# geoeo/ORB_SLAM3_V1.0

Measured on AMD Instinct MI355X. Metric: frames/sec ORB extract+match, 752x480 8-level 1000-feat; bit-exact kp/desc, higher is better.
Workload: dtype u8

## Files before the change

orb_slam3_v1.0_amd/csrc/fast_common.h:

```cpp
#pragma once
#include <hip/hip_runtime.h>
#include <stdint.h>

namespace orbfe {

constexpr int kFastTW = 64, kFastTH = 32;

constexpr int kFusedPyramidMinFrames = 0;

__device__ __forceinline__ bool arc9(uint32_t m)
{
    uint32_t m2 = m | (m << 16);
    uint32_t r = m2 & (m2 >> 1);
    r &= r >> 2;
    r &= r >> 4;
    r &= m2 >> 8;
    return (r & 0xffffu) != 0;
}

__device__ __forceinline__ bool corner_at_global(const uint8_t* __restrict__ img, int pitch, int x, int y, int th)
{
    const int8_t dy[16] = {3, 3, 2, 1, 0, -1, -2, -3, -3, -3, -2, -1, 0, 1, 2, 3};
    const int8_t dx[16] = {0, 1, 2, 3, 3, 3, 2, 1, 0, -1, -2, -3, -3, -3, -2, -1};
    const int v = img[(size_t)y * pitch + x];
    uint32_t mb = 0, md = 0;
#pragma unroll
    for (int k = 0; k < 16; k++) {
        const int d = (int)img[(size_t)(y + dy[k]) * pitch + x + dx[k]] - v;
        mb |= (uint32_t)(d > th) << k;
        md |= (uint32_t)(d < -th) << k;
    }
    return arc9(mb) || arc9(md);
}

}
```

orb_slam3_v1.0_amd/csrc/kernels_fast.hip:

```cpp
#include <cstdlib>

#include "launch.h"
#include "device_math.h"
#include "fast_common.h"

namespace orbfe {

constexpr int kImgW = kFastTW + 8, kImgH = kFastTH + 8;
constexpr int kScH = kFastTH + 2;
constexpr int kScW = kFastTW + 2;
constexpr int kScPitch = kImgW;
constexpr int kScoreOfs = 3 * kImgW + 3;
constexpr int kMaxTileCand = (kFastTW / 2) * (kFastTH / 2);
constexpr int kTmpH = kFastTH + 4;
constexpr int kQCap = 2304;
static_assert(kQCap >= kScH * kScW && kQCap % 2 == 0, "stage A geometry");

typedef unsigned short u16x2 __attribute__((ext_vector_type(2)));


__device__ __forceinline__ unsigned long long mask_le_u32(uint32_t x, uint32_t bound)
{
    unsigned long long m;
    asm("v_cmp_le_u32_e64 %0, %1, %2" : "=s"(m) : "v"(x), "s"(bound));
    return m;
}

__device__ __forceinline__ unsigned long long mask_ge_u32(uint32_t x, uint32_t bound)
{
    unsigned long long m;
    asm("v_cmp_ge_u32_e64 %0, %1, %2" : "=s"(m) : "v"(x), "s"(bound));
    return m;
}
__device__ __forceinline__ unsigned long long mask_gt_u32(uint32_t a, uint32_t b)
{
    unsigned long long m;
    asm("v_cmp_gt_u32_e64 %0, %1, %2" : "=s"(m) : "v"(a), "v"(b));
    return m;
}
__device__ __forceinline__ uint32_t select_by_mask(unsigned long long mask, uint32_t a, uint32_t b)
{
    uint32_t r;
    asm("v_cndmask_b32_e64 %0, %1, %2, %3" : "=v"(r) : "v"(b), "v"(a), "s"(mask));
    return r;
}
__device__ __forceinline__ void masked_lds_add(unsigned long long mask, uint32_t addr, uint32_t v)
{
    unsigned long long save;
    asm volatile("s_and_saveexec_b64 %0, %1\n\tds_add_u32 %2, %3\n\ts_mov_b64 exec, %0" : "=&s"(save) : "s"(mask), "v"(addr), "v"(v) : "scc", "memory");
}
__device__ __forceinline__ void masked_lds_write_b32(unsigned long long mask, uint32_t addr, uint32_t v)
{
    unsigned long long save;
    asm volatile("s_and_saveexec_b64 %0, %1\n\tds_write_b32 %2, %3\n\ts_mov_b64 exec, %0" : "=&s"(save) : "s"(mask), "v"(addr), "v"(v) : "scc", "memory");
}
__device__ __forceinline__ unsigned long long mask_lt_i32(uint32_t a, int b, bool vbound = false)
{
    unsigned long long m;
    if (vbound) asm("v_cmp_lt_i32_e64 %0, %1, %2" : "=s"(m) : "v"(a), "v"(b));
    else asm("v_cmp_lt_i32_e64 %0, %1, %2" : "=s"(m) : "v"(a), "s"(b));
    return m;
}
__device__ __forceinline__ void masked_lds_write_b8(unsigned long long mask, uint32_t addr, uint32_t v)
{
    unsigned long long save;
    asm volatile("s_and_saveexec_b64 %0, %1\n\tds_write_b8 %2, %3\n\ts_mov_b64 exec, %0" : "=&s"(save) : "s"(mask), "v"(addr), "v"(v) : "scc", "memory");
}
__device__ __forceinline__ void masked_lds_write_b16(unsigned long long mask, uint32_t addr, uint32_t v)
{
    unsigned long long save;
    asm volatile("s_and_saveexec_b64 %0, %1\n\tds_write_b16 %2, %3\n\ts_mov_b64 exec, %0" : "=&s"(save) : "s"(mask), "v"(addr), "v"(v) : "scc", "memory");
}
__device__ __forceinline__ void lds_add(uint32_t* addr, uint32_t v)
{
    asm volatile("ds_add_u32 %0, %1" : : "v"((uint32_t)(uintptr_t)addr), "v"(v) : "memory");
}

__device__ __forceinline__ uint32_t lds_add_rtn(uint32_t* addr, uint32_t v)
{
    uint32_t old;
    asm volatile("ds_add_rtn_u32 %0, %1, %2\n\ts_waitcnt lgkmcnt(0)" : "=&v"(old) : "v"((uint32_t)(uintptr_t)addr), "v"(v) : "memory");
    return old;
}

__device__ __forceinline__ uint32_t min16(uint32_t a, uint32_t b)
{
    uint32_t r;
    asm("v_min_u16 %0, %1, %2" : "=v"(r) : "v"(a), "v"(b));
    return r;
}
__device__ __forceinline__ uint32_t max16(uint32_t a, uint32_t b)
{
    uint32_t r;
    asm("v_max_u16 %0, %1, %2" : "=v"(r) : "v"(a), "v"(b));
    return r;
}
__device__ __forceinline__ uint32_t sub16(uint32_t a, uint32_t b)
{
    uint32_t r;
    asm("v_sub_u16 %0, %1, %2" : "=v"(r) : "v"(a), "v"(b));
    return r;
}
__device__ __forceinline__ uint32_t maxi16(uint32_t a, uint32_t b)
{
    uint32_t r;
    asm("v_max_i16 %0, %1, %2" : "=v"(r) : "v"(a), "v"(b));
    return r;
}

template <bool DARK>
__device__ __forceinline__ uint32_t arc_extreme(const uint32_t (&p)[16])
{
    auto lo = [](uint32_t a, uint32_t b) { return DARK ? max16(a, b) : min16(a, b); };
    auto hi = [](uint32_t a, uint32_t b) { return DARK ? min16(a, b) : max16(a, b); };
    uint32_t m2[8], m4[8], a[8];
#pragma unroll
    for (int j = 0; j < 8; j++) m2[j] = lo(p[2 * j + 1], p[(2 * j + 2) & 15]);
#pragma unroll
    for (int j = 0; j < 8; j++) m4[j] = lo(m2[j], m2[(j + 1) & 7]);
#pragma unroll
    for (int j = 0; j < 8; j++) {
        const uint32_t core = lo(m4[j], m4[(j + 2) & 7]);
        a[j] = lo(core, hi(p[2 * j], p[(2 * j + 9) & 15]));
    }
#pragma unroll
    for (int st = 4; st >= 1; st >>= 1)
#pragma unroll
        for (int k = 0; k < st; k++) a[k] = hi(a[k], a[k + st]);
    return a[0];
}
__device__ __forceinline__ uint32_t arc_max_of_min(const uint32_t (&p)[16]) { return arc_extreme<false>(p); }
__device__ __forceinline__ uint32_t arc_min_of_max(const uint32_t (&p)[16]) { return arc_extreme<true>(p); }

__device__ __forceinline__ unsigned long long mask_th_i16(int th, uint32_t m)
{
    unsigned long long r;
    asm("v_cmp_lt_i16_e64 %0, %1, %2" : "=s"(r) : "s"(th), "v"(m));
    return r;
}

__device__ __forceinline__ int queue_slot1(uint32_t m, int th, unsigned long long mask, uint32_t entry, int stepV, int qNext)
{
    unsigned long long save;
    uint32_t tmp;
    int cnt;
    asm volatile("v_cmp_lt_i16_e32 vcc, %8, %3\n\t"
                 "s_and_b64 vcc, vcc, %4\n\t"
                 "s_and_saveexec_b64 %0, vcc\n\t"
                 "v_mbcnt_lo_u32_b32 %1, vcc_lo, 0\n\t"
                 "v_mbcnt_hi_u32_b32 %1, vcc_hi, %1\n\t"
                 "v_mad_i32_i24 %1, %1, %6, %7\n\t"
                 "ds_write_b16 %1, %5\n\t"
                 "s_mov_b64 exec, %0\n\t"
                 "s_bcnt1_i32_b64 %2, vcc"
                 : "=&s"(save), "=&v"(tmp), "=s"(cnt)
                 : "v"(m), "s"(mask), "v"(entry), "v"(stepV), "s"(qNext), "s"(th)
                 : "vcc", "scc", "memory");
    return cnt;
}

template <int MODE, bool BUILD>
__global__ __launch_bounds__(256) void fast_blur_kernel(const PipelineDesc* __restrict__ P,
                                                        const uint32_t* __restrict__ tileInfo, int tileBase,
                                                        const uint32_t* __restrict__ tabs,
                                                        const uint8_t* __restrict__ gray0, size_t gray0FrameStride,
// ... 41 lines not shown
    const int tid = threadIdx.x;
    const int lane = tid & 63;
    if (tid < 4) sCnt[tid] = 0;
    if (tid < 3) sQ[tid] = 0;
    if (tid < kFastTH) sRow[tid] = 0;

    int bXa = 0, bNX = 0, bYa = 0, bNY = 0;
    uint32_t bXt = 0, bYt = 0;
    if constexpr (BUILD) {
        const uint32_t* own = tabs + L.ownOff;
        const int tX = (int)(ti & 0xfffu), tY = (int)((ti >> 12) & 0xfffu);
        bXa = (int)own[tX];
        bNX = (int)own[tX + 1] - bXa;
        bYa = (int)own[L.tilesX + 1 + tY];
        bNY = (int)own[L.tilesX + 2 + tY] - bYa;
        const LevelDesc& D = P->lv[l + 1];
        if (lane < bNX) bXt = tabs[D.xtabOff + (size_t)(bXa + lane)];
        if (lane < bNY) bYt = tabs[D.ytabOff + (size_t)(bYa + lane)];
    }

    if (aligned) {
        if (tid < 14 * (kImgW / 4)) {
            const int r0 = tid / (kImgW / 4);
            const int c4 = tid - r0 * (kImgW / 4);
            const int gx = x0 - 4 + 4 * c4;
            const bool colIn = gx >= 0 && gx < w;
            uint32_t wv[3];
            if (y0 >= 4 && y0 + kFastTH + 4 <= h) {
                uint32_t off = __umul24((unsigned)(y0 - 4 + r0), (unsigned)spitch) + (unsigned)gx;
                const uint32_t step = 14u * (unsigned)spitch;
#pragma unroll
                for (int k = 0; k < 3; k++) {
                    wv[k] = 0;
                    if (colIn && r0 + 14 * k < kImgH) wv[k] = *reinterpret_cast<const uint32_t*>(src + off);
                    off += step;
                }
            } else {
#pragma unroll
                for (int k = 0; k < 3; k++) {
                    const int r = r0 + 14 * k;
                    wv[k] = 0;
                    if (colIn && r < kImgH)
                        wv[k] = *reinterpret_cast<const uint32_t*>(src + (size_t)reflect_near(y0 - 4 + r, h) * spitch + gx);
                }
            }
#pragma unroll
            for (int k = 0; k < 3; k++) {
                const int r = r0 + 14 * k;
                if (colIn && r < kImgH) *reinterpret_cast<uint32_t*>(&sImg[r][4 * c4]) = wv[k];
            }
        }
        const int cR = w - x0 + 4;
        const bool patchL = x0 == 0, patchR = cR + 1 < kImgW;
        if (patchL || patchR) {
            __syncthreads();
            if (tid < kImgH) {
                if (patchL) {
                    sImg[tid][2] = sImg[tid][6];
                    sImg[tid][3] = sImg[tid][5];
                }
            } else if (tid >= 64 && tid < 64 + kImgH) {
                if (patchR) {
                    sImg[tid - 64][cR] = sImg[tid - 64][cR - 2];
                    sImg[tid - 64][cR + 1] = sImg[tid - 64][cR - 3];
                }
            }
        }
    } else {
        for (int e = tid; e < kImgH * (kImgW / 4); e += 256) {
            const int r = e / (kImgW / 4);
            const int c4 = e - r * (kImgW / 4);
            const uint8_t* row = src + (size_t)reflect_near(y0 - 4 + r, h) * spitch;
            uint32_t wv = 0;
#pragma unroll
            for (int i = 0; i < 4; i++) wv |= (uint32_t)row[reflect_near(x0 - 4 + 4 * c4 + i, w)] << (8 * i);
            *reinterpret_cast<uint32_t*>(&sImg[r][4 * c4]) = wv;
        }
    }
    __syncthreads();

    if constexpr (BUILD) {
        static_assert(kFastTH == 32, "eight owned rows per wave at most");
        const LevelDesc& D = P->lv[l + 1];
        if (lane < bNX && bNY > 0) {
            const uint32_t wx = bXt >> 16, wxc = 2048u - wx;
            const uint8_t* sp = &sImg[0][0] + ((int)(bXt & 0xffffu) - (x0 - 4));
            uint8_t* dcol = ws + D.imgOff + (size_t)f * D.imgFrameStride + (uint32_t)(bYa * D.pitch + bXa + lane);
            const int q = __builtin_amdgcn_readfirstlane(tid >> 6);
            uint32_t top[8], bot[8], wy[8];
#pragma unroll
            for (int k = 0; k < 8; k++) {
                const uint32_t yt = (uint32_t)__builtin_amdgcn_readlane((int)bYt, min(q + 4 * k, bNY - 1));
                const uint8_t* pr = sp + ((int)(yt & 0xffffu) - (y0 - 4)) * kImgW;
                wy[k] = yt >> 16;
                top[k] = __umul24(pr[0], wxc) + __umul24(pr[1], wx);
                bot[k] = __umul24(pr[kImgW], wxc) + __umul24(pr[kImgW + 1], wx);
            }
#pragma unroll
            for (int k = 0; k < 8; k++) {
                const uint32_t v = __umul24(top[k], 2048u - wy[k]) + __umul24(bot[k], wy[k]) + (1u << 21);
                if (q + 4 * k < bNY) dcol[(uint32_t)((q + 4 * k) * D.pitch)] = (uint8_t)(v >> 22);
            }
        }
    }

    if constexpr ((MODE & 1) != 0) {
    for (int e = tid; e < (kTmpH / 2) * (kFastTW / 4); e += 256) {
        const int j = e / (kFastTW / 4);
        const int xl = (e - j * (kFastTW / 4)) * 4;
        uint32_t o[2][4];
#pragma unroll
        for (int half = 0; half < 2; half++) {
            const uint32_t* rowp = reinterpret_cast<const uint32_t*>(&sImg[2 * j + half + 2][xl]);
            const uint32_t w0 = rowp[0], w1 = rowp[1], w2 = rowp[2];
            o[half][0] = __builtin_amdgcn_udot4(w1, 0x00163E58u, __builtin_amdgcn_udot4(w0, 0x3E160000u, 0u, false), false);
            o[half][1] = __builtin_amdgcn_udot4(w1, 0x163E583Eu, __builtin_amdgcn_udot4(w0, 0x16000000u, 0u, false), false);
            o[half][2] = __builtin_amdgcn_udot4(w2, 0x00000016u, __builtin_amdgcn_udot4(w1, 0x3E583E16u, 0u, false), false);
            o[half][3] = __builtin_amdgcn_udot4(w2, 0x0000163Eu, __builtin_amdgcn_udot4(w1, 0x583E1600u, 0u, false), false);
        }
        uint4 pk;
        pk.x = o[0][0] | (o[1][0] << 16);
        pk.y = o[0][1] | (o[1][1] << 16);
        pk.z = o[0][2] | (o[1][2] << 16);
        pk.w = o[0][3] | (o[1][3] << 16);
        *reinterpret_cast<uint4*>(&sTmp[j][xl]) = pk;
    }
    __syncthreads();
    }

    const int wv = __builtin_amdgcn_readfirstlane(tid >> 6);
    if (wv >= 2) {
        if constexpr ((MODE & 2) != 0)
            for (int e = tid - 128; e < (kScH + 1) * (kScPitch / 4); e += 128) reinterpret_cast<uint32_t*>(&sScore[0][0])[e] = 0;
        if constexpr ((MODE & 1) != 0) {
            uint8_t* dst = ws + L.blurOff + (size_t)f * L.blurFrameStride;
            const int dpitch = L.pitch;
            const int xl = (tid & 15) * 4;
#pragma unroll 1
            for (int yp = (tid - 128) >> 4; yp < kFastTH / 2; yp += 8) {
                const int gy = y0 + 2 * yp, gx = x0 + xl;
                if (gy < h && gx < w) {
                    const uint4 p0 = *reinterpret_cast<const uint4*>(&sTmp[yp][xl]);
                    const uint4 p1 = *reinterpret_cast<const uint4*>(&sTmp[yp + 1][xl]);
                    const uint4 p2 = *reinterpret_cast<const uint4*>(&sTmp[yp + 2][xl]);
                    const uint32_t c0[4] = {p0.x, p0.y, p0.z, p0.w}, c1[4] = {p1.x, p1.y, p1.z, p1.w}, c2[4] = {p2.x, p2.y, p2.z, p2.w};
                    uint32_t ev[4], od[4];
#pragma unroll
                    for (int i = 0; i < 4; i++) {
                        const u16x2 a = __builtin_bit_cast(u16x2, c0[i]), b = __builtin_bit_cast(u16x2, c1[i]), c = __builtin_bit_cast(u16x2, c2[i]);
                        uint32_t acc = __builtin_amdgcn_udot2(a, __builtin_bit_cast(u16x2, 0x003E0016u), 32768u, false);
                        acc = __builtin_amdgcn_udot2(b, __builtin_bit_cast(u16x2, 0x003E0058u), acc, false);
                        ev[i] = __builtin_amdgcn_udot2(c, __builtin_bit_cast(u16x2, 0x00000016u), acc, false);
                        acc = __builtin_amdgcn_udot2(a, __builtin_bit_cast(u16x2, 0x00160000u), 32768u, false);
                        acc = __builtin_amdgcn_udot2(b, __builtin_bit_cast(u16x2, 0x0058003Eu), acc, false);
                        od[i] = __builtin_amdgcn_udot2(c, __builtin_bit_cast(u16x2, 0x0016003Eu), acc, false);
                    }
                    const uint32_t outE = __builtin_amdgcn_perm(ev[1], ev[0], 0x0c0c0602u) |
                                          (__builtin_amdgcn_perm(ev[3], ev[2], 0x0c0c0602u) << 16);
                    const uint32_t outO = __builtin_amdgcn_perm(od[1], od[0], 0x0c0c0602u) |
                                          (__builtin_amdgcn_perm(od[3], od[2], 0x0c0c0602u) << 16);
                    uint8_t* drow = dst + (size_t)gy * dpitch;
                    const bool odd = gy + 1 < h;
                    if (gx + 3 < w) {
                        *reinterpret_cast<uint32_t*>(drow + gx) = outE;
                        if (odd) *reinterpret_cast<uint32_t*>(drow + dpitch + gx) = outO;
                    } else {
                        for (int i = 0; gx + i < w; i++) {
                            drow[gx + i] = (uint8_t)(outE >> (8 * i));
                            if (odd) drow[dpitch + gx + i] = (uint8_t)(outO >> (8 * i));
                        }
                    }
                }
            }
        }
    } else if constexpr ((MODE & 2) != 0) {
        constexpr int kRowsA = kScH / 2;
        static_assert(2 * kRowsA == kScH && kScW == 66, "stage A geometry");
        const int R0 = wv ? 3 + kRowsA : 3;
        const int cLo = max(3, kEdge + 1 - (x0 - 4)), cHi = min(kScW + 2, w - kEdge - 1 - (x0 - 4));
        const int rLo = max(3, kEdge + 1 - (y0 - 4)), rHi = min(kScH + 2, h - kEdge - 1 - (y0 - 4));
        const uint32_t cSpan = (uint32_t)max(cHi - cLo, -1), rSpan = (uint32_t)max(rHi - rLo, -1);
        const bool anyValid = cSpan != 0xffffffffu && rSpan != 0xffffffffu;
        const unsigned long long colOK = anyValid ? mask_le_u32((uint32_t)(lane + 3 - cLo), cSpan) : 0ull;
        const int qStep = wv ? -2 : 2;
// ... 130 lines not shown
            if (mPre == 0) continue;
            const uint8_t* sp = &sScore[0][0] + (e - kScoreOfs);
            const uint32_t sc = sp[0];
            const uint32_t n0 = max16(max16((uint32_t)sp[-kScPitch - 1], (uint32_t)sp[-kScPitch]), (uint32_t)sp[-kScPitch + 1]);
            const uint32_t n1 = max16(max16((uint32_t)sp[-1], (uint32_t)sp[1]), (uint32_t)sp[kScPitch - 1]);
            const uint32_t n2 = max16((uint32_t)sp[kScPitch], (uint32_t)sp[kScPitch + 1]);
            const uint32_t nmax = max16(max16(n0, n1), n2);
            const unsigned long long mHi = mask_ge_u32(sc, (uint32_t)iniTh);
            const unsigned long long mKeep = mPre & mask_gt_u32(sc, nmax);
            const unsigned long long mPreHi = mPre & mHi, mKeepHi = mKeep & mHi;
            nPreW += (uint32_t)__popcll(mPre);
            nPreHiW += (uint32_t)__popcll(mPreHi);
            nKeepHiW += (uint32_t)__popcll(mKeepHi);
            masked_lds_add(mPre, rowLds + 4u * oy, select_by_mask(mHi, 0x10001u, 1u));
            if (mKeep) {
                uint32_t wbase = 0;
                if (lane == 0) wbase = lds_add_rtn(&sCnt[0], (uint32_t)__popcll(mKeep));
                wbase = __builtin_amdgcn_readfirstlane(wbase);
                const uint32_t rank = __builtin_amdgcn_mbcnt_hi((uint32_t)(mKeep >> 32), __builtin_amdgcn_mbcnt_lo((uint32_t)mKeep, 0u));
                masked_lds_write_b32(mKeep, candLds + 4u * (wbase + rank), pack_cand(x0 + (int)ox, y0 + (int)oy, (int)sc));
            }
        }
        if (lane == 0) {
            if (nPreW) lds_add(&sCnt[2], nPreW);
            if (nPreHiW) lds_add(&sCnt[3], nPreHiW);
            if (nKeepHiW) lds_add(&sCnt[1], nKeepHiW);
        }
        asm volatile("s_waitcnt lgkmcnt(0)" ::: "memory");
    }
    __syncthreads();

    }

    if (tid < kFastTH) {
        const uint32_t v = sRow[tid];
        tileRows[((size_t)f * P->totalTiles + tile) * kFastTH + tid] = (uint16_t)((v & 0xffu) | ((v >> 16) << 8));
    }

    uint32_t* cnt = counters + ((size_t)f * nL + l) * kCntWords;
    const uint32_t nTile = sCnt[0];
    if (tid == 0) {
        uint32_t base = 0;
        if constexpr ((MODE & 256) != 0) base = (uint32_t)tile * 8u;
        else if (nTile) base = atomicAdd(&cnt[kCntCand], nTile);
        if (sCnt[1]) atomicAdd(&cnt[kCntHigh], sCnt[1]);
        if (sCnt[2]) atomicAdd(&cnt[kCntPreLow], sCnt[2]);
        if (sCnt[3]) atomicAdd(&cnt[kCntPreHigh], sCnt[3]);
        sBase = base;
    }
    __syncthreads();
    if (nTile) {
        const uint32_t base = sBase;
        uint32_t* out = cand + L.candOff + (size_t)f * L.candCap;
        for (uint32_t i = tid; i < nTile; i += 256) {
            if (base + i < (uint32_t)L.candCap) out[base + i] = sCand[i];
            else atomicOr(&cnt[kCntStatus], (uint32_t)kFlagCandOverflow);
        }
    }
}

void fast_tiles_for(int w, int h, int* tx, int* ty)
{
    *tx = (w + kFastTW - 1) / kFastTW;
    *ty = (h + kFastTH - 1) / kFastTH;
}

bool fast_next_level_fits(const uint32_t* xtab, const uint32_t* ytab, int sw, int sh, int dw, int dh, uint32_t* own)
{
    int tx, ty;
    fast_tiles_for(sw, sh, &tx, &ty);
    bool ok = true;
    auto fill = [&](const uint32_t* tab, int srcN, int dstN, int tile, int nTiles, uint32_t* o) {
        int p = 0;
        for (int t = 0; t <= nTiles; t++) {
            while (p < dstN && (int)(tab[p] & 0xffffu) < t * tile) p++;
            o[t] = (uint32_t)(t == nTiles ? dstN : p);
            if (t > 0 && o[t] - o[t - 1] > 64u) ok = false;
        }
        for (int i = 0; i < dstN; i++)
            if ((int)(tab[i] & 0xffffu) + 1 > srcN - 1 || (i > 0 && (tab[i] & 0xffffu) < (tab[i - 1] & 0xffffu))) ok = false;
    };
    fill(xtab, sw, dw, kFastTW, tx, own);
    fill(ytab, sh, dh, kFastTH, ty, own + tx + 1);
    return ok;
}

uint32_t fast_tile_info(int level, int tileX, int tileY) { return ((uint32_t)level << 24) | ((uint32_t)tileY << 12) | (uint32_t)tileX; }

void launch_fast_blur(hipStream_t s, int frames, int tileBase, int nTiles, bool buildNext, const PipelineDesc* dP,
                      const uint32_t* dTileInfo, const uint32_t* dTabs, const uint8_t* gray0, size_t gray0FrameStride, int gray0Pitch,
                      int gray0Aligned4, uint8_t* ws, uint32_t* cand, uint32_t* counters, uint16_t* tileRows)
{
    dim3 block(256);
    dim3 grid(frames, nTiles);
    if (buildNext) {
        hipLaunchKernelGGL((fast_blur_kernel<3, true>), grid, block, 0, s, dP, dTileInfo, tileBase, dTabs, gray0, gray0FrameStride,
                           gray0Pitch, gray0Aligned4, ws, cand, counters, tileRows);
        return;
    }
#define ORBFE_LAUNCH_FB(M)                                                                                                      \
    hipLaunchKernelGGL((fast_blur_kernel<M, false>), grid, block, 0, s, dP, dTileInfo, tileBase, dTabs, gray0, gray0FrameStride, \
                       gray0Pitch, gray0Aligned4, ws, cand, counters, tileRows)
#ifdef ORBFE_ABLATION
    static const int mode = [] {
        const char* e = getenv("ORBFE_FAST_MODE");
        return e ? atoi(e) & 1023 : 3;
    }();
    switch (mode) {
    case 0: ORBFE_LAUNCH_FB(0); break;
    case 1: ORBFE_LAUNCH_FB(1); break;
    case 2: ORBFE_LAUNCH_FB(2); break;
    case 6: ORBFE_LAUNCH_FB(6); break;
    case 10: ORBFE_LAUNCH_FB(10); break;
    case 26: ORBFE_LAUNCH_FB(26); break;
    case 67: ORBFE_LAUNCH_FB(67); break;
    case 195: ORBFE_LAUNCH_FB(195); break;
    case 259: ORBFE_LAUNCH_FB(259); break;
    case 515: ORBFE_LAUNCH_FB(515); break;
    case 42: ORBFE_LAUNCH_FB(42); break;
    default: ORBFE_LAUNCH_FB(3); break;
    }
#else
    ORBFE_LAUNCH_FB(3);
#endif
#undef ORBFE_LAUNCH_FB
}

}
```

orb_slam3_v1.0_amd/csrc/orbfe_host.cpp:

```cpp
#include <atomic>
#include <cmath>
#include <cstdio>
#include <cstdlib>
#include <cstring>
#include <map>
#include <mutex>
#include <new>
#include <condition_variable>
#include <functional>
#include <string>
#include <thread>
#include <vector>

#include "launch.h"
#include "fast_common.h"
#include "match.h"
#include "match_common.h"
#include "match_proj.h"
#include "keyframe.h"
#include "prep.h"
#include "vocab.h"

using namespace orbfe;

namespace {

constexpr int kEventSets = 128;

size_t align_up(size_t v, size_t a) { return (v + a - 1) / a * a; }

const char* kStageNames[ORBFE_NUM_STAGES] = {"pyramid_resize", "fast_nms_blur",
                                             "quadtree", "orient_brief", "total"};

struct ChainBlocks {
    uint8_t *dIn = nullptr, *hIn = nullptr, *dOut = nullptr, *hOut = nullptr;
};

template <class Key>
struct GraphCache {
    struct Entry {
        Key key;
        hipGraphExec_t exec;
    };
    std::vector<Entry> entries;
    hipGraphExec_t find(const Key& key) const
    {
        for (const Entry& e : entries)
            if (memcmp(&e.key, &key, sizeof key) == 0) return e.exec;
        return nullptr;
    }
    void insert(const Key& key, hipGraphExec_t exec, size_t bound)
    {
        if (entries.size() >= bound) drop();
        entries.push_back({key, exec});
    }
    void drop()
    {
        for (Entry& e : entries)
            if (e.exec) (void)hipGraphExecDestroy(e.exec);
        entries.clear();
    }
};

}

struct orbfe_map;
struct orbfe_stream;

struct orbfe_handle {
    orbfe_params prm{};
    int device = 0;
    int nLevels = 0;
    double scaleFactorD = 0.0;
    float sf[kMaxLevels]{}, inv[kMaxLevels]{}, sig2[kMaxLevels]{}, invSig2[kMaxLevels]{};
    PipelineDesc P{};
    PipelineDesc* dP = nullptr;
    int maxBatch = 1;
    int maxNodeCap = 0;

    uint8_t* ws = nullptr;
    size_t wsBytes = 0;
    uint32_t* dCand = nullptr;
    uint16_t* dNodeOf = nullptr;
    size_t candWordsPerBatch = 0;
    uint32_t* dCounters = nullptr;
    uint32_t* dLvlKp = nullptr;
    uint16_t* dTileRows = nullptr;
    uint8_t* dQtScratch = nullptr;
    uint32_t* dTabs = nullptr;
    uint32_t* dTileInfo = nullptr;
    bool pyrFits[kMaxLevels]{};
    bool fusedFits[kMaxLevels]{};
    int fusedMinFrames = kFusedPyramidMinFrames;
    bool fusedSplitOnly = false;
    float* dSf = nullptr;

    uint8_t* dIn = nullptr;
    int dInPitch = 0;
    uint8_t* hIn = nullptr;
    uint8_t* dOutBlock = nullptr;
    uint8_t* hOutBlock = nullptr;
    size_t outBlockBytes = 0, offStatus = 0, offPer = 0, offKp = 0, offDesc = 0;
    orbfe_keypoint* dKp = nullptr;
    uint8_t* dDesc = nullptr;
    int* dN = nullptr;
    int* dStatus = nullptr;
    int* dPer = nullptr;
    orbfe_keypoint* hKp = nullptr;
    uint8_t* hDesc = nullptr;
    int* hN = nullptr;
    int* hStatus = nullptr;
    int* hPer = nullptr;
    std::map<int, hipGraphExec_t> graphs;
    bool useGraph = true;
    int graphCaptures = 0, captureFailures = 0;
    int captureFailStreak = 0;

    hipStream_t stream = nullptr;
    bool timing = false;
    hipEvent_t ev[kEventSets][ORBFE_NUM_STAGES]{};
    int evHead = 0, evCount = 0;

    const uint8_t* lastGray = nullptr;
    size_t lastStride = 0;
    int lastPitch = 0, lastBatch = 0;

    MatchScratch match;

    struct TrackKey {
        int Mb, inPitch, gridCols, gridRows, farPoints;
        float minX, minY, invW, invH, th, nnRatio, thFar;
        const void* map;
    };
    MatchScratch trackMatch;
    ChainBlocks trk;
    int trkCapM = 0;
    GraphCache<TrackKey> trackGraphs;
    struct RefKey {
        int inPitch, levelsup, checkOri;
        float nnRatio;
        unsigned long long vocabSerial;
    };
    ChainBlocks ref;
    int refCapFlags = 0;
    GraphCache<RefKey> refGraphs;
    struct IniKey {
        int inPitch, gridCols, gridRows, window, checkOri;
        float minX, minY, invW, invH, nnRatio;
        unsigned long long frameSerial;
    };
    ChainBlocks ini;
    int iniCapN1 = -1;
    size_t iniScratchBytes = 0;
    GraphCache<IniKey> iniGraphs;
    std::mutex mu;
    std::string err;
    std::vector<orbfe_map*> maps;
    std::vector<orbfe_stream*> rings;

    hipEvent_t evExtract = nullptr, evMatch = nullptr;
    hipStream_t extractStream = nullptr, matchStream = nullptr;
    bool extractUsed = false, matchUsed = false;
};

namespace {

int fail_hip(orbfe_handle* h, hipError_t e, const char* what, int line)
{
    char buf[256];
    snprintf(buf, sizeof buf, "%s failed at orbfe_host.cpp:%d: %s", what, line, hipGetErrorString(e));
    if (h) h->err = buf;
    return ORBFE_ERR_HIP;
}

#define HIPCHK(h, call)                                                   \
    do {                                                                  \
        hipError_t e_ = (call);                                           \
// ... 244 lines not shown
    h->candWordsPerBatch = candOff;

    std::vector<uint32_t> tabs(tabOff ? tabOff : 1, 0);
    for (int l = 1; l < nL; l++) {
        fill_resize_table(tabs, P.lv[l].xtabOff, P.lv[l - 1].w, P.lv[l].w);
        fill_resize_table(tabs, P.lv[l].ytabOff, P.lv[l - 1].h, P.lv[l].h);
    }

    for (int l = 1; l < nL; l++)
        if (pyramid_level_fits(tabs.data() + P.lv[l].xtabOff, tabs.data() + P.lv[l].ytabOff, P.lv[l - 1].w, P.lv[l - 1].h, P.lv[l].w,
                               P.lv[l].h))
            h->pyrFits[l] = true;
    for (int l = 1; l < nL; l++)
        h->fusedFits[l] = fast_next_level_fits(tabs.data() + P.lv[l].xtabOff, tabs.data() + P.lv[l].ytabOff, P.lv[l - 1].w, P.lv[l - 1].h,
                                               P.lv[l].w, P.lv[l].h, tabs.data() + P.lv[l - 1].ownOff) && h->pyrFits[l];

#define CREATE_CHK(call)                                                  \
    do {                                                                  \
        hipError_t e_ = (call);                                           \
        if (e_ != hipSuccess) {                                           \
            int rc_ = e_ == hipErrorOutOfMemory ? ORBFE_ERR_OUT_OF_MEMORY : ORBFE_ERR_HIP; \
            destroy_impl(h);                                              \
            return rc_;                                                   \
        }                                                                 \
    } while (0)

    CREATE_CHK(hipStreamCreateWithFlags(&h->stream, hipStreamNonBlocking));
    CREATE_CHK(hipMalloc(&h->dP, sizeof(PipelineDesc)));
    CREATE_CHK(hipMalloc(&h->ws, h->wsBytes + 256));
    CREATE_CHK(hipMalloc(&h->dCand, candOff * sizeof(uint32_t)));
    CREATE_CHK(hipMalloc(&h->dNodeOf, candOff * sizeof(uint16_t)));
    CREATE_CHK(hipMalloc(&h->dCounters, B * nL * kCntWords * sizeof(uint32_t)));
    CREATE_CHK(hipMalloc(&h->dLvlKp, B * (size_t)P.kpCapFrame * sizeof(uint32_t)));
    CREATE_CHK(hipMalloc(&h->dTileRows, B * (size_t)P.totalTiles * 32 * sizeof(uint16_t)));
    if (quadtree_scratch_bytes_per_block(h->maxNodeCap))
        CREATE_CHK(hipMalloc(&h->dQtScratch, quadtree_scratch_bytes_per_block(h->maxNodeCap) * B * nL));
    CREATE_CHK(hipMalloc(&h->dTabs, tabs.size() * sizeof(uint32_t)));
    {
        std::vector<uint32_t> info((size_t)P.totalTiles);
        for (int l = 0; l < nL; l++)
            for (int ty = 0; ty < P.lv[l].tilesY; ty++)
                for (int tx = 0; tx < P.lv[l].tilesX; tx++) info[P.lv[l].tileBase + ty * P.lv[l].tilesX + tx] = fast_tile_info(l, tx, ty);
        CREATE_CHK(hipMalloc(&h->dTileInfo, info.size() * sizeof(uint32_t)));
        CREATE_CHK(copy_sync(h->dTileInfo, info.data(), info.size() * sizeof(uint32_t), hipMemcpyHostToDevice, h->stream));
    }
    CREATE_CHK(hipMalloc(&h->dSf, kMaxLevels * sizeof(float)));
    CREATE_CHK(copy_sync(h->dSf, h->sf, kMaxLevels * sizeof(float), hipMemcpyHostToDevice, h->stream));
    CREATE_CHK(copy_sync(h->dP, &P, sizeof P, hipMemcpyHostToDevice, h->stream));
    CREATE_CHK(copy_sync(h->dTabs, tabs.data(), tabs.size() * sizeof(uint32_t), hipMemcpyHostToDevice, h->stream));

    h->dInPitch = (int)align_up((size_t)p->image_width, kPitchAlign);
    const size_t inFrame = (size_t)h->dInPitch * p->image_height;
    const size_t cap = (size_t)P.kpCapFrame;
    CREATE_CHK(hipMalloc(&h->dIn, inFrame * B));
    CREATE_CHK(hipHostMalloc(&h->hIn, inFrame * B));
    {
        size_t off = 0;
        auto take = [&](size_t bytes) { const size_t o = off; off = align_up(off + bytes, 256); return o; };
        take(B * sizeof(int));
        h->offStatus = take(B * sizeof(int));
        h->offPer = take(B * nL * sizeof(int));
        h->offKp = take(B * cap * sizeof(orbfe_keypoint));
        h->offDesc = take(B * cap * ORBFE_DESC_BYTES);
        h->outBlockBytes = off;
    }
    CREATE_CHK(hipMalloc(&h->dOutBlock, h->outBlockBytes));
    CREATE_CHK(hipHostMalloc(&h->hOutBlock, h->outBlockBytes));
    h->dN = reinterpret_cast<int*>(h->dOutBlock);
    h->dStatus = reinterpret_cast<int*>(h->dOutBlock + h->offStatus);
    h->dPer = reinterpret_cast<int*>(h->dOutBlock + h->offPer);
    h->dKp = reinterpret_cast<orbfe_keypoint*>(h->dOutBlock + h->offKp);
    h->dDesc = h->dOutBlock + h->offDesc;
    h->hN = reinterpret_cast<int*>(h->hOutBlock);
    h->hStatus = reinterpret_cast<int*>(h->hOutBlock + h->offStatus);
    h->hPer = reinterpret_cast<int*>(h->hOutBlock + h->offPer);
    h->hKp = reinterpret_cast<orbfe_keypoint*>(h->hOutBlock + h->offKp);
    h->hDesc = h->hOutBlock + h->offDesc;
#ifdef ORBFE_DIAG
    h->useGraph = getenv("ORBFE_NO_GRAPH") == nullptr;
    if (const char* e = getenv("ORBFE_FUSED_PYRAMID")) {
        h->fusedMinFrames = atoi(e) ? 1 : 0;
        h->fusedSplitOnly = atoi(e) == 2;
    }
#endif
    CREATE_CHK(hipEventCreateWithFlags(&h->evExtract, hipEventDisableTiming));
    CREATE_CHK(hipEventCreateWithFlags(&h->evMatch, hipEventDisableTiming));
    h->match.busy = h->evMatch;
    for (auto& set : h->ev)
        for (auto& e : set) CREATE_CHK(hipEventCreate(&e));
#undef CREATE_CHK
    *out = h;
    return ORBFE_OK;
}

void orbfe_destroy(orbfe_handle* h) { destroy_impl(h); }

int orbfe_get_levels(const orbfe_handle* h) { return h ? h->nLevels : 0; }
float orbfe_get_scale_factor(const orbfe_handle* h) { return h ? (float)h->scaleFactorD : 0.f; }

int orbfe_get_scale_tables(const orbfe_handle* h, float* sf, float* inv, float* s2, float* is2)
{
    if (!h) return ORBFE_ERR_INVALID_ARG;
    for (int i = 0; i < h->nLevels; i++) {
        if (sf) sf[i] = h->sf[i];
        if (inv) inv[i] = h->inv[i];
        if (s2) s2[i] = h->sig2[i];
        if (is2) is2[i] = h->invSig2[i];
    }
    return ORBFE_OK;
}

int orbfe_get_level_info(const orbfe_handle* h, int* fpl, int* lw, int* lh)
{
    if (!h) return ORBFE_ERR_INVALID_ARG;
    for (int i = 0; i < h->nLevels; i++) {
        if (fpl) fpl[i] = h->P.lv[i].nFeatures;
        if (lw) lw[i] = h->P.lv[i].w;
        if (lh) lh[i] = h->P.lv[i].h;
    }
    return ORBFE_OK;
}

int orbfe_max_keypoints(const orbfe_handle* h) { return h ? h->P.kpCapFrame : 0; }

int orbfe_set_stage_timing(orbfe_handle* h, int enabled)
{
    if (!h) return ORBFE_ERR_INVALID_ARG;
    h->timing = enabled != 0;
    h->evHead = h->evCount = 0;
    return ORBFE_OK;
}

int orbfe_get_stage_ms(orbfe_handle* h, float ms[ORBFE_NUM_STAGES], int* n_calls)
{
    if (!h || !ms || !n_calls) return ORBFE_ERR_INVALID_ARG;
    HIPCHK(h, hipSetDevice(h->device));
    for (int s = 0; s < ORBFE_NUM_STAGES; s++) ms[s] = 0.f;
    const int n = h->evCount < kEventSets ? h->evCount : kEventSets;
    for (int i = 0; i < n; i++) {
        hipEvent_t* e = h->ev[i];
        HIPCHK(h, hipEventSynchronize(e[ORBFE_NUM_STAGES - 1]));
        for (int s = 0; s + 1 < ORBFE_NUM_STAGES; s++) {
            float t = 0.f;
            HIPCHK(h, hipEventElapsedTime(&t, e[s], e[s + 1]));
            ms[s] += t;
        }
        float t = 0.f;
        HIPCHK(h, hipEventElapsedTime(&t, e[0], e[ORBFE_NUM_STAGES - 1]));
        ms[ORBFE_NUM_STAGES - 1] += t;
    }
    *n_calls = n;
    return ORBFE_OK;
}

static int extract_chain(orbfe_handle* h, const uint8_t* d_gray, size_t frame_stride, int pitch, int batch,
                         orbfe_keypoint* d_kp, uint8_t* d_desc, int* d_n, int* d_per, int* d_status, void* stream_);

int orbfe_extract_batch_device(orbfe_handle* h, const uint8_t* d_gray, size_t frame_stride, int pitch,
                               int batch, orbfe_keypoint* d_kp, uint8_t* d_desc, int* d_n, int* d_per,
                               void* stream_)
{
    if (!h) return ORBFE_ERR_INVALID_ARG;
    std::lock_guard<std::mutex> lk(h->mu);
    return extract_chain(h, d_gray, frame_stride, pitch, batch, d_kp, d_desc, d_n, d_per, nullptr, stream_);
}

}

static int extract_chain(orbfe_handle* h, const uint8_t* d_gray, size_t frame_stride, int pitch, int batch,
                         orbfe_keypoint* d_kp, uint8_t* d_desc, int* d_n, int* d_per, int* d_status, void* stream_)
{
    if (!h || !d_gray || !d_kp || !d_desc || !d_n) return ORBFE_ERR_INVALID_ARG;
    if (batch < 1 || batch > h->maxBatch || pitch < h->prm.image_width || pitch >= (1 << 24)) return ORBFE_ERR_INVALID_ARG;
    const int aligned4 = ((reinterpret_cast<uintptr_t>(d_gray) | (uintptr_t)pitch | (uintptr_t)frame_stride) & 3u) == 0;
    const size_t rowEnd = aligned4 ? (size_t)((h->prm.image_width + 3) & ~3) : (size_t)h->prm.image_width;
    if (batch > 1 && frame_stride < (size_t)pitch * (h->prm.image_height - 1) + rowEnd) return ORBFE_ERR_INVALID_ARG;
    if ((size_t)pitch * (h->prm.image_height - 1) + (size_t)((h->prm.image_width + 3) & ~3) >= (size_t)0x7ffffff0u)
        return ORBFE_ERR_INVALID_ARG;
    HIPCHK(h, hipSetDevice(h->device));
    hipStream_t s = stream_ ? (hipStream_t)stream_ : h->stream;
    hipStreamCaptureStatus capturing = hipStreamCaptureStatusNone;
    if (hipStreamIsCapturing(s, &capturing) != hipSuccess) (void)hipGetLastError();
    if (capturing == hipStreamCaptureStatusNone) {
        const int rc = scratch_acquire(h, h->extractUsed, h->extractStream, h->evExtract, s);
        if (rc != ORBFE_OK) return rc;
    }
    const PipelineDesc& P = h->P;
    const int nL = P.nLevels;
    hipEvent_t* ev = nullptr;
    if (h->timing) {
        ev = h->ev[h->evHead];
        h->evHead = (h->evHead + 1) % kEventSets;
        h->evCount++;
    }
    const bool fused = h->fusedMinFrames > 0 && batch >= h->fusedMinFrames && nL > 1;
    const bool chainPyr = !fused && (long long)batch * nL <= 64 && !ev && nL > 1;
    if (!chainPyr) HIPCHK(h, hipMemsetAsync(h->dCounters, 0, (size_t)batch * nL * kCntWords * sizeof(uint32_t), s));
    if (ev) HIPCHK(h, hipEventRecord(ev[0], s));
    for (int l = 1; chainPyr && l < nL;) {
        const int left = nL - l;
        const int depth = left >= 5 ? 2 : std::min(left, 3);
        launch_pyramid_chain(s, batch, h->dP, P, l - 1, depth, d_gray, frame_stride, pitch, h->ws, h->dTabs,
                             l == 1 ? h->dCounters : nullptr, nL * kCntWords);
        l += depth;
    }
    auto pyramid_level = [&](int l) {
        const LevelDesc& S = P.lv[l - 1];
        const LevelDesc& D = P.lv[l];
        if (h->pyrFits[l] && (l > 1 || aligned4)) {
            launch_pyramid_level(s, batch, h->dP, l, D.w, D.h, d_gray, frame_stride, pitch, h->ws, h->dTabs);
            return;
        }
        const uint8_t* src = l == 1 ? d_gray : h->ws + S.imgOff;
        const size_t sstride = l == 1 ? frame_stride : S.imgFrameStride;
        const int spitch = l == 1 ? pitch : S.pitch;
        launch_resize(s, batch, src, sstride, S.w, S.h, spitch, l == 1 ? aligned4 : 1, h->ws + D.imgOff, D.imgFrameStride, D.w, D.h,
                      D.pitch, h->dTabs + D.xtabOff, h->dTabs + D.ytabOff);
    };
    for (int l = chainPyr || (fused && !h->fusedSplitOnly) ? nL : 1; l < nL; l++) pyramid_level(l);
    if (ev) HIPCHK(h, hipEventRecord(ev[1], s));
    if (fused) {
        for (int l = 0; l < nL; l++) {
            const bool build = l + 1 < nL && h->fusedFits[l + 1] && !h->fusedSplitOnly;
            launch_fast_blur(s, batch, P.lv[l].tileBase, P.lv[l].tilesX * P.lv[l].tilesY, build, h->dP, h->dTileInfo, h->dTabs, d_gray,
                             frame_stride, pitch, aligned4, h->ws, h->dCand, h->dCounters, h->dTileRows);
            if (l + 1 < nL && !build && !h->fusedSplitOnly) pyramid_level(l + 1);
        }
    } else {
        launch_fast_blur(s, batch, 0, P.totalTiles, false, h->dP, h->dTileInfo, h->dTabs, d_gray, frame_stride, pitch, aligned4, h->ws,
                         h->dCand, h->dCounters, h->dTileRows);
    }
    if (ev) HIPCHK(h, hipEventRecord(ev[2], s));
    launch_quadtree(s, batch, nL, h->maxNodeCap, h->dP, h->dCand, h->dNodeOf, h->dCounters, h->dLvlKp, d_gray, frame_stride,
                    pitch, h->ws, h->dTileRows, h->dQtScratch);
    if (ev) HIPCHK(h, hipEventRecord(ev[3], s));
    int kpBase[kMaxLevels];
    for (int l = 0; l < nL; l++) kpBase[l] = P.lv[l].kpBase;
    launch_orient_brief(s, batch, P.kpCapFrame, h->dP, d_gray, frame_stride, pitch, h->ws, h->dCounters, h->dLvlKp,
                        d_kp, d_desc, d_n, d_per, d_status, kpBase, nL);
    if (ev) HIPCHK(h, hipEventRecord(ev[4], s));
    HIPCHK(h, hipGetLastError());
    h->lastGray = d_gray;
    h->lastStride = frame_stride;
    h->lastPitch = pitch;
    h->lastBatch = batch;
    if (capturing == hipStreamCaptureStatusNone) return extract_scratch_release(h, s);
    return ORBFE_OK;
}

extern "C" {

static int check_device_flags(orbfe_handle* h, int batch)
{
    for (int b = 0; b < batch; b++)
        if (h->hStatus[b]) {
            char buf[128];
            snprintf(buf, sizeof buf, "device guard flags 0x%x at frame %d", (unsigned)h->hStatus[b], b);
            h->err = buf;
            return ORBFE_ERR_INTERNAL;
        }
    return ORBFE_OK;
}

static int extract_host_enqueue(orbfe_handle* h, int batch, int inPitch, hipStream_t s)
{
    const int nL = h->nLevels;
    const size_t inFrame = (size_t)h->dInPitch * h->prm.image_height;
    const size_t cap = (size_t)h->P.kpCapFrame;
    const int rc = extract_chain(h, h->dIn, inFrame, inPitch, batch, h->dKp, h->dDesc, h->dN, h->dPer, h->dStatus, s);
    if (rc != ORBFE_OK) return rc;
    if (batch == h->maxBatch) {
        HIPCHK(h, hipMemcpyAsync(h->hOutBlock, h->dOutBlock, h->outBlockBytes, hipMemcpyDeviceToHost, s));
    } else {
        HIPCHK(h, hipMemcpyAsync(h->hN, h->dN, batch * sizeof(int), hipMemcpyDeviceToHost, s));
        HIPCHK(h, hipMemcpyAsync(h->hStatus, h->dStatus, batch * sizeof(int), hipMemcpyDeviceToHost, s));
        HIPCHK(h, hipMemcpyAsync(h->hPer, h->dPer, (size_t)batch * nL * sizeof(int), hipMemcpyDeviceToHost, s));
        HIPCHK(h, hipMemcpyAsync(h->hKp, h->dKp, batch * cap * sizeof(orbfe_keypoint), hipMemcpyDeviceToHost, s));
        HIPCHK(h, hipMemcpyAsync(h->hDesc, h->dDesc, batch * cap * ORBFE_DESC_BYTES, hipMemcpyDeviceToHost, s));
    }
    return ORBFE_OK;
}

}

namespace {

struct CaptureStream {
    hipStream_t s = nullptr;
    bool capturing = false;
    bool begin()
    {
        if (hipStreamCreateWithFlags(&s, hipStreamNonBlocking) != hipSuccess) {
            s = nullptr;
            (void)hipGetLastError();
            return false;
        }
        if (hipStreamBeginCapture(s, hipStreamCaptureModeThreadLocal) != hipSuccess) {
            (void)hipGetLastError();
            return false;
        }
        capturing = true;
        return true;
    }
    hipGraph_t end()
    {
        hipGraph_t g = nullptr;
        if (capturing) {
            capturing = false;
            if (hipStreamEndCapture(s, &g) != hipSuccess) {
                (void)hipGetLastError();
// ... 2202 lines not shown
```

Before: 223,900.

## Build next pyramid level with banded separable walk and merge tail-level FAST launches

The fused pyramid build inside the FAST kernel now gives each wave a contiguous band of destination rows. It computes horizontal interpolations once per staged source row and reuses them across adjacent output rows, instead of recomputing both rows per output with strided stores. Custom mad24/store asm is used, and the host fit check now also verifies the band stays within the staged rows. On the host side, the last levels' FAST launches are merged into a single launch after their pyramid levels are built, which cuts launch count. The merged launch adds serialization of the remaining pyramid builds before the tail FAST work.

Result: no change. 224,100 (median of 6 runs) (+0.1%).

```diff
diff --git a/orb_slam3_v1.0_amd/csrc/fast_common.h b/orb_slam3_v1.0_amd/csrc/fast_common.h
--- a/orb_slam3_v1.0_amd/csrc/fast_common.h
+++ b/orb_slam3_v1.0_amd/csrc/fast_common.h
@@ -7,6 +7,7 @@
 constexpr int kFastTW = 64, kFastTH = 32;
 
 constexpr int kFusedPyramidMinFrames = 0;
+constexpr int kFusedTailLevels = 0;
 
 __device__ __forceinline__ bool arc9(uint32_t m)
 {
diff --git a/orb_slam3_v1.0_amd/csrc/kernels_fast.hip b/orb_slam3_v1.0_amd/csrc/kernels_fast.hip
--- a/orb_slam3_v1.0_amd/csrc/kernels_fast.hip
+++ b/orb_slam3_v1.0_amd/csrc/kernels_fast.hip
@@ -1,3 +1,4 @@
+#include <algorithm>
 #include <cstdlib>
 
 #include "launch.h"
@@ -15,6 +16,8 @@
 constexpr int kTmpH = kFastTH + 4;
 constexpr int kQCap = 2304;
 static_assert(kQCap >= kScH * kScW && kQCap % 2 == 0, "stage A geometry");
+constexpr int kBuildSpan = 10;
+static_assert(kBuildSpan <= kImgH, "the walk stays inside the staged rows");
 
 typedef unsigned short u16x2 __attribute__((ext_vector_type(2)));
 
@@ -81,6 +84,29 @@
     uint32_t old;
     asm volatile("ds_add_rtn_u32 %0, %1, %2\n\ts_waitcnt lgkmcnt(0)" : "=&v"(old) : "v"((uint32_t)(uintptr_t)addr), "v"(v) : "memory");
     return old;
+}
+
+__device__ __forceinline__ uint32_t mul24(uint32_t a, uint32_t b)
+{
+    uint32_t r;
+    asm("v_mul_u32_u24_e32 %0, %1, %2" : "=v"(r) : "v"(a), "v"(b));
+    return r;
+}
+__device__ __forceinline__ uint32_t mad24(uint32_t a, uint32_t b, uint32_t c)
+{
+    uint32_t r;
+    asm("v_mad_u32_u24 %0, %1, %2, %3" : "=v"(r) : "v"(a), "v"(b), "v"(c));
+    return r;
+}
+__device__ __forceinline__ uint32_t mad24_s(uint32_t a, uint32_t sb, uint32_t c)
+{
+    uint32_t r;
+    asm("v_mad_u32_u24 %0, %1, %2, %3" : "=v"(r) : "v"(a), "s"(sb), "v"(c));
+    return r;
+}
+__device__ __forceinline__ void store_b8_row(uint8_t* row, uint32_t off, uint32_t v)
+{
+    asm volatile("global_store_byte %0, %1, %2" : : "v"(off), "v"(v), "s"(row) : "memory");
 }
 
 __device__ __forceinline__ uint32_t min16(uint32_t a, uint32_t b)
@@ -288,24 +314,34 @@
     if constexpr (BUILD) {
         static_assert(kFastTH == 32, "eight owned rows per wave at most");
         const LevelDesc& D = P->lv[l + 1];
-        if (lane < bNX && bNY > 0) {
+        const int q = __builtin_amdgcn_readfirstlane(tid >> 6);
+        const int band = (bNY + 3) >> 2;
+        const int rEnd = min(q * band + band, bNY);
+        int k = q * band;
+        if (k < rEnd && lane < bNX) {
             const uint32_t wx = bXt >> 16, wxc = 2048u - wx;
-            const uint8_t* sp = &sImg[0][0] + ((int)(bXt & 0xffffu) - (x0 - 4));
-            uint8_t* dcol = ws + D.imgOff + (size_t)f * D.imgFrameStride + (uint32_t)(bYa * D.pitch + bXa + lane);
-            const int q = __builtin_amdgcn_readfirstlane(tid >> 6);
-            uint32_t top[8], bot[8], wy[8];
-#pragma unroll
-            for (int k = 0; k < 8; k++) {
-                const uint32_t yt = (uint32_t)__builtin_amdgcn_readlane((int)bYt, min(q + 4 * k, bNY - 1));
-                const uint8_t* pr = sp + ((int)(yt & 0xffffu) - (y0 - 4)) * kImgW;
-                wy[k] = yt >> 16;
-                top[k] = __umul24(pr[0], wxc) + __umul24(pr[1], wx);
-                bot[k] = __umul24(pr[kImgW], wxc) + __umul24(pr[kImgW + 1], wx);
-            }
-#pragma unroll
-            for (int k = 0; k < 8; k++) {
-                const uint32_t v = __umul24(top[k], 2048u - wy[k]) + __umul24(bot[k], wy[k]) + (1u << 21);
-                if (q + 4 * k < bNY) dcol[(uint32_t)((q + 4 * k) * D.pitch)] = (uint8_t)(v >> 22);
+            uint32_t yt = (uint32_t)__builtin_amdgcn_readlane((int)bYt, k);
+            int ys = (int)(yt & 0xffffu) - (y0 - 4);
+            const int s0 = min(ys, kImgH - kBuildSpan);
+            const uint8_t* sp = &sImg[0][0] + ((int)(bXt & 0xffffu) - (x0 - 4)) + s0 * kImgW;
+            uint8_t* drow = ws + D.imgOff + (size_t)f * D.imgFrameStride + (uint32_t)((bYa + k) * D.pitch);
+            const uint32_t dcol = (uint32_t)(bXa + lane);
+            uint32_t half;
+            asm("v_mov_b32 %0, 0x200000" : "=v"(half));
+            uint32_t hs[kBuildSpan];
+#pragma unroll
+            for (int j = 0; j < kBuildSpan; j++) hs[j] = mad24(sp[j * kImgW + 1], wx, mul24(sp[j * kImgW], wxc));
+#pragma unroll
+            for (int j = 0; j < kBuildSpan - 1; j++) {
+                if (k < rEnd && ys == s0 + j) {
+                    const uint32_t wy = yt >> 16;
+                    const uint32_t v = mad24_s(hs[j + 1], wy, mad24_s(hs[j], 2048u - wy, half));
+                    store_b8_row(drow, dcol, v >> 22);
+                    drow += D.pitch;
+                    k++;
+                    yt = (uint32_t)__builtin_amdgcn_readlane((int)bYt, k);
+                    ys = (int)(yt & 0xffffu) - (y0 - 4);
+                }
             }
         }
     }
@@ -602,6 +638,20 @@
     };
     fill(xtab, sw, dw, kFastTW, tx, own);
     fill(ytab, sh, dh, kFastTH, ty, own + tx + 1);
+    for (int i = 1; i < dh; i++)
+        if ((ytab[i] & 0xffffu) <= (ytab[i - 1] & 0xffffu)) ok = false;
+    const uint32_t* oy = own + tx + 1;
+    for (int t = 0; ok && t < ty; t++) {
+        const int a = (int)oy[t], n = (int)oy[t + 1] - a;
+        if (n > kFastTH) ok = false;
+        const int band = (n + 3) / 4;
+        for (int q = 0; ok && q < 4 && q * band < n; q++) {
+            const int first = (int)(ytab[a + q * band] & 0xffffu), last = (int)(ytab[a + std::min(q * band + band, n) - 1] & 0xffffu);
+            const int top = t * kFastTH - 4;
+            const int s0 = std::min(first - top, kImgH - kBuildSpan);
+            if (first - top < 4 || last + 1 - top - s0 > kBuildSpan - 1) ok = false;
+        }
+    }
     return ok;
 }
 
diff --git a/orb_slam3_v1.0_amd/csrc/orbfe_host.cpp b/orb_slam3_v1.0_amd/csrc/orbfe_host.cpp
--- a/orb_slam3_v1.0_amd/csrc/orbfe_host.cpp
+++ b/orb_slam3_v1.0_amd/csrc/orbfe_host.cpp
@@ -93,6 +93,7 @@
     bool fusedFits[kMaxLevels]{};
     int fusedMinFrames = kFusedPyramidMinFrames;
     bool fusedSplitOnly = false;
+    int fusedTailLevels = kFusedTailLevels;
     float* dSf = nullptr;
 
     uint8_t* dIn = nullptr;
@@ -503,6 +504,7 @@
         h->fusedMinFrames = atoi(e) ? 1 : 0;
         h->fusedSplitOnly = atoi(e) == 2;
     }
+    if (const char* e = getenv("ORBFE_FUSED_TAIL")) h->fusedTailLevels = std::max(0, atoi(e));
 #endif
     CREATE_CHK(hipEventCreateWithFlags(&h->evExtract, hipEventDisableTiming));
     CREATE_CHK(hipEventCreateWithFlags(&h->evMatch, hipEventDisableTiming));
@@ -641,12 +643,16 @@
     for (int l = chainPyr || (fused && !h->fusedSplitOnly) ? nL : 1; l < nL; l++) pyramid_level(l);
     if (ev) HIPCHK(h, hipEventRecord(ev[1], s));
     if (fused) {
-        for (int l = 0; l < nL; l++) {
-            const bool build = l + 1 < nL && h->fusedFits[l + 1] && !h->fusedSplitOnly;
+        const int last = std::max(1, nL - 1 - h->fusedTailLevels);
+        for (int l = 0; l < last; l++) {
+            const bool build = h->fusedFits[l + 1] && !h->fusedSplitOnly;
             launch_fast_blur(s, batch, P.lv[l].tileBase, P.lv[l].tilesX * P.lv[l].tilesY, build, h->dP, h->dTileInfo, h->dTabs, d_gray,
                              frame_stride, pitch, aligned4, h->ws, h->dCand, h->dCounters, h->dTileRows);
-            if (l + 1 < nL && !build && !h->fusedSplitOnly) pyramid_level(l + 1);
-        }
+            if (!build && !h->fusedSplitOnly) pyramid_level(l + 1);
+        }
+        for (int l = last + 1; l < nL && !h->fusedSplitOnly; l++) pyramid_level(l);
+        launch_fast_blur(s, batch, P.lv[last].tileBase, P.totalTiles - P.lv[last].tileBase, false, h->dP, h->dTileInfo, h->dTabs, d_gray,
+                         frame_stride, pitch, aligned4, h->ws, h->dCand, h->dCounters, h->dTileRows);
     } else {
         launch_fast_blur(s, batch, 0, P.totalTiles, false, h->dP, h->dTileInfo, h->dTabs, d_gray, frame_stride, pitch, aligned4, h->ws,
                          h->dCand, h->dCounters, h->dTileRows);
```
